# kvignesh1420/rlap

Hardware: AMD Instinct MI355X
Metric: eliminated-vertices/sec (higher is better)
Workload: dtype f64

## Files before the change

### rlap_amd/csrc/rlap_core.h

```cpp
#pragma once
#include <stdint.h>

#if defined(__HIPCC__)
#define RLAP_HD __host__ __device__ __forceinline__
#define RLAP_HD_NOINLINE __host__ __device__ __noinline__
#else
#define RLAP_HD inline
#define RLAP_HD_NOINLINE inline
#endif

namespace rlap {

enum { OV_RANDOM = 0, OV_DEGREE = 1, OV_COARSEN = 2 };
enum { ON_ASC = 0, ON_DESC = 1, ON_RANDOM = 2 };

enum {
    ST_OK = 0,
    ST_NOT_SYMMETRIC = 1,
    ST_INDEX_RANGE = 2,
    ST_BAD_ARG = 3,
    ST_POOL_OVERFLOW = 4,
    ST_LOG_OVERFLOW = 5,
    ST_RNG_OVERFLOW = 6,
    ST_OUT_OVERFLOW = 7,
    ST_HIP_ERROR = 8,
    ST_TOO_LARGE = 9,
    ST_INTERNAL = 10,
    ST_FLOW_SCRATCH = 12,
    ST_FLOW_REORDER = 13,
};

RLAP_HD uint64_t mix64(uint64_t z) {
    z += 0x9E3779B97F4A7C15ull;
    z = (z ^ (z >> 30)) * 0xBF58476D1CE4E5B9ull;
    z = (z ^ (z >> 27)) * 0x94D049BB133111EBull;
    return z ^ (z >> 31);
}
RLAP_HD uint64_t keyed_order_base(uint64_t seed, int64_t vertex, int phase) {
    return mix64(seed ^ mix64(2ull * (uint64_t)vertex + (uint64_t)phase));
}
RLAP_HD uint64_t keyed_order_key(uint64_t base, int64_t nbr) { return mix64(base ^ mix64((uint64_t)nbr)); }

enum { RNG_STREAM = 0, RNG_COUNTER = 1 };
RLAP_HD double frontier_uniform(uint64_t seed, int64_t vertex, int64_t j) {
    const uint64_t z = mix64(mix64((seed ^ 0x66726F6E74696572ull) ^ mix64((uint64_t)vertex)) ^ mix64((uint64_t)j));
    return (double)(z >> 11) * 1.1102230246251565e-16;
}

constexpr int CHUNK0 = 8;
RLAP_HD int ilog2_u32(unsigned q) {
#if defined(__HIP_DEVICE_COMPILE__)
    return 31 - __clz((int)q);
#else
    int c = 0;
    while (q > 1u) { q >>= 1; ++c; }
    return c;
#endif
}
RLAP_HD int chunk_of(int a) {
    return ilog2_u32((unsigned)a / CHUNK0 + 1u);
}
RLAP_HD int chunk_start(int c) { return CHUNK0 * ((1 << c) - 1); }
RLAP_HD int chunk_cap(int c) { return CHUNK0 << c; }

RLAP_HD int pq_list_of(int key, int n) { return key <= n ? key : n + key / n; }

RLAP_HD void pq_op(int& key, int& mv, int n, int delta, int opnum) {
    if (delta < 0 && key == 1) return;
    int ol = pq_list_of(key, n), nl = pq_list_of(key + delta, n);
    key += delta;
    if (ol != nl) mv = opnum;
}

struct SRec {
    double key;
    int32_t idx;
    int32_t aux;
};

template <bool GREATER>
RLAP_HD bool srec_less(const SRec& a, const SRec& b) {
    return GREATER ? (a.key > b.key) : (a.key < b.key);
}

template <class T, class Less, class P>
RLAP_HD void gs_adjust_heap(P a, int first, int hole, int len, T value, Less less) {
    const int top = hole;
    int child = hole;
    while (child < (len - 1) / 2) {
        child = 2 * (child + 1);
        if (less(a[first + child], a[first + child - 1])) child--;
        a[first + hole] = a[first + child];
        hole = child;
    }
    if ((len & 1) == 0 && child == (len - 2) / 2) {
        child = 2 * (child + 1);
        a[first + hole] = a[first + child - 1];
        hole = child - 1;
    }
    int parent = (hole - 1) / 2;
    while (hole > top && less(a[first + parent], value)) {
        a[first + hole] = a[first + parent];
        hole = parent;
        parent = (hole - 1) / 2;
    }
    a[first + hole] = value;
}

template <class T, class Less, class P>
RLAP_HD void gs_heap_sort(P a, int first, int last, Less less) {
    int len = last - first;
    if (len >= 2) {
        int parent = (len - 2) / 2;
        while (true) {
            T v = a[first + parent];
            gs_adjust_heap<T>(a, first, parent, len, v, less);
            if (parent == 0) break;
            parent--;
        }
    }
    int l = last;
    while (l - first > 1) {
        --l;
        T v = a[l];
        a[l] = a[first];
        gs_adjust_heap<T>(a, first, 0, l - first, v, less);
    }
}

template <class T, class Less, class P>
RLAP_HD void gs_introsort_loop(P a, int n, Less less) {
    if (n <= 16) return;
    int depth0 = 0;
    for (unsigned q = (unsigned)n; q > 1u; q >>= 1) ++depth0;
    depth0 *= 2;
    int stk_first[72], stk_last[72], stk_depth[72];
    int sp = 0;
    stk_first[0] = 0; stk_last[0] = n; stk_depth[0] = depth0; sp = 1;
    while (sp > 0) {
        --sp;
        int first = stk_first[sp], last = stk_last[sp], depth = stk_depth[sp];
        while (last - first > 16) {
            if (depth == 0) { gs_heap_sort<T>(a, first, last, less); break; }
            --depth;
            int ia = first + 1, ib = first + (last - first) / 2, ic = last - 1;
            int pick;
            if (less(a[ia], a[ib])) {
                if (less(a[ib], a[ic])) pick = ib;
                else if (less(a[ia], a[ic])) pick = ic;
                else pick = ia;
            } else if (less(a[ia], a[ic])) pick = ia;
            else if (less(a[ib], a[ic])) pick = ic;
            else pick = ib;
            { T t = a[first]; a[first] = a[pick]; a[pick] = t; }
            T pv = a[first];
            int f = first + 1, l = last;
            while (true) {
                while (less(a[f], pv)) ++f;
                --l;
                while (less(pv, a[l])) --l;
                if (!(f < l)) break;
                T t = a[f]; a[f] = a[l]; a[l] = t;
                ++f;
            }
            int cut = f;
            stk_first[sp] = cut; stk_last[sp] = last; stk_depth[sp] = depth; ++sp;
            last = cut;
        }
    }
}

template <class T, class Less, class P>
RLAP_HD void gs_introsort_loop_small(P a, int n, Less less) {
    if (n <= 16) return;
    int depth = 0;
    for (unsigned q = (unsigned)n; q > 1u; q >>= 1) ++depth;
    depth *= 2;
    int first = 0, last = n;
    while (last - first > 16) {
        if (depth == 0) { gs_heap_sort<T>(a, first, last, less); break; }
        --depth;
        int ia = first + 1, ib = first + (last - first) / 2, ic = last - 1;
        int pick;
        if (less(a[ia], a[ib])) {
            if (less(a[ib], a[ic])) pick = ib;
            else if (less(a[ia], a[ic])) pick = ic;
            else pick = ia;
        } else if (less(a[ia], a[ic])) pick = ia;
        else if (less(a[ib], a[ic])) pick = ic;
        else pick = ib;
        { T t = a[first]; a[first] = a[pick]; a[pick] = t; }
        T pv = a[first];
        int f = first + 1, l = last;
        while (true) {
            while (less(a[f], pv)) ++f;
            --l;
            while (less(pv, a[l])) --l;
            if (!(f < l)) break;
            T t = a[f]; a[f] = a[l]; a[l] = t;
            ++f;
        }
        if (last - f > 16) first = f; else last = f;
    }
}
template <class T, class Less, class P>
RLAP_HD void gs_insertion_sort(P a, int n, Less less) {
    for (int i = 1; i < n; ++i) {
        T v = a[i];
        int j = i - 1;
        while (j >= 0 && less(v, a[j])) { a[j + 1] = a[j]; --j; }
        a[j + 1] = v;
    }
}

template <class T, class Less, class P>
RLAP_HD void gs_std_sort_small(P a, int n, Less less) {
    if (n < 2) return;
    gs_introsort_loop_small<T>(a, n, less);
    gs_insertion_sort<T>(a, n, less);
}

template <class T, class Less, class P>
RLAP_HD void gs_std_sort(P a, int n, Less less) {
    if (n < 2) return;
    gs_introsort_loop<T>(a, n, less);
    gs_insertion_sort<T>(a, n, less);
}

template <bool GREATER>
struct SRecLess {
    RLAP_HD bool operator()(const SRec& x, const SRec& y) const { return GREATER ? (x.key > y.key) : (x.key < y.key); }
};

template <bool GREATER, class P>
RLAP_HD void ss_heap_sort(P a, int first, int last) { gs_heap_sort<SRec>(a, first, last, SRecLess<GREATER>()); }

template <bool GREATER, class P>
RLAP_HD void std_sort_emul(P a, int n) { gs_std_sort<SRec>(a, n, SRecLess<GREATER>()); }

RLAP_HD double keyed_order_dkey(uint64_t base, int64_t nbr) { return (double)(keyed_order_key(base, nbr) >> 12); }

struct GraphDesc {
    int32_t vbase;
    int32_t n;
    int64_t t;
    int32_t bucket_base;
    int32_t pad0;
    int32_t pad1;
    int32_t scr_base;
    int32_t scr_cap;
    int32_t minlist;
    int32_t push_cnt;
    int32_t n_elim;
    int32_t status;
    int64_t n_draws;
    int64_t out_rows;
    int32_t flow_base;
    int32_t resume;
    int32_t narrow;
    int32_t narrow_rounds;
    int32_t pool_cur;
    int32_t pool_end;
};

struct ColBuf {
    SRec* rec;
    int32_t* a_slot; int32_t* a_nbr; int32_t* a_twin; double* a_val;
    int32_t* b_slot; int32_t* b_nbr; int32_t* b_twin; double* b_val;
    double* cum; double* newv;
    int32_t* ksel; int32_t* t_key; int32_t* t_mv; int32_t* t_of;
};

struct alignas(16) Slot {
    double val;
    int32_t nbr;
    int32_t twin;
};
struct alignas(16) VRec {
    int32_t key;
    int32_t pqpos;
    int32_t app_cnt;
    int32_t app_chunk;
};
struct Arrays {
    const int32_t* colptr;
    Slot* e;
    int32_t slot_cap;
    int32_t* pool_top;
    VRec* vr;
    int32_t* ocur; int32_t* oend;
    int32_t* bs_cnt; int32_t* bs_alloc;
    int32_t* bs_dir;
    int32_t* bs_v; int32_t* bs_id;
    int32_t* bs_pool_top; int32_t bs_pool_cap;
    const int32_t* orig_order;
    const double* rng; int64_t rng_len;
    const int64_t* perm;
    int32_t o_v; int32_t o_n;
    uint64_t shuffle_seed;
    int32_t rng_mode;
    int32_t vbase;
};
RLAP_HD double arr_uniform(const Arrays& A, int64_t draw, int32_t vertex, int32_t j) {
    return A.rng_mode == RNG_COUNTER ? frontier_uniform(A.shuffle_seed, (int64_t)(vertex - A.vbase), (int64_t)j) : A.rng[draw];
}
RLAP_HD bool keyed_order(const Arrays& A) { return A.o_n == ON_RANDOM || A.o_v == OV_COARSEN; }

#if defined(__HIP_DEVICE_COMPILE__)
RLAP_HD int32_t pool_take(int32_t* top, int32_t cnt) { return atomicAdd(top, cnt); }
#else
RLAP_HD int32_t pool_take(int32_t* top, int32_t cnt) { int32_t r = *top; *top = r + cnt; return r; }
#endif

RLAP_HD int32_t col_append(const Arrays& A, int32_t k) {
    int32_t a = A.vr[k].app_cnt;
    int c = chunk_of(a);
    int cs = chunk_start(c);
    if (a == cs) {
        int32_t need = 1 + chunk_cap(c);
        int32_t base = pool_take(A.pool_top, need);
        if (base < 0 || base > A.slot_cap - need) return -1;
        A.e[base].nbr = A.vr[k].app_chunk;
        A.vr[k].app_chunk = base;
    }
    A.vr[k].app_cnt = a + 1;
    return A.vr[k].app_chunk + 1 + (a - cs);
}

RLAP_HD int32_t serial_gather(const Arrays& A, int32_t v, const ColBuf& B, int32_t cap) {
    int32_t len = 0;
    int32_t a = A.vr[v].app_cnt;
    if (a > 0) {
        int32_t base = A.vr[v].app_chunk;
        int c = chunk_of(a - 1);
        int32_t idx = a - 1;
        while (idx >= 0) {
            int32_t cs = chunk_start(c);
            for (int32_t t = idx; t >= cs; --t) {
                int32_t s = base + 1 + (t - cs);
                double val = A.e[s].val;
                if (val > 0) {
                    if (len < cap) { B.a_slot[len] = s; B.a_nbr[len] = A.e[s].nbr; B.a_val[len] = val; B.a_twin[len] = A.e[s].twin; }
                    ++len;
                }
            }
            idx = cs - 1;
            base = A.e[base].nbr;
            --c;
        }
    }
    for (int32_t s = A.colptr[v + 1] - 1; s >= A.colptr[v]; --s) {
        double val = A.e[s].val;
        if (val > 0) {
            if (len < cap) { B.a_slot[len] = s; B.a_nbr[len] = A.e[s].nbr; B.a_val[len] = val; B.a_twin[len] = A.e[s].twin; }
            ++len;
        }
    }
    return len;
}

constexpr int SQUEEZE_PASSES = 2;

template <class F>
RLAP_HD void col_for_each_slot(const Arrays& A, int32_t v, F f) {
    const int32_t a = A.vr[v].app_cnt;
    if (a > 0) {
        int32_t base = A.vr[v].app_chunk;
        int c = chunk_of(a - 1);
        int32_t idx = a - 1;
        while (idx >= 0 && base >= 0) {
            const int32_t cs = chunk_start(c);
            for (int32_t t = idx; t >= cs; --t) f(base + 1 + (t - cs));
            idx = cs - 1;
            base = A.e[base].nbr;
            --c;
        }
    }
    for (int32_t s = A.colptr[v + 1] - 1; s >= A.colptr[v]; --s) f(s);
}
#if defined(__HIPCC__)
template <class Sink>
__device__ __forceinline__ int32_t wave_col_live(const Arrays& A, int32_t v, int lane, Sink sink) {
    const uint64_t lt = lane == 0 ? 0ull : (~0ull >> (64 - lane));
    int32_t len = 0;
    auto piece = [&](int32_t hi, int32_t lo) {
        for (int32_t s0 = hi; s0 >= lo; s0 -= 64) {
            const int32_t s = s0 - lane;
            Slot g = {};
            if (s >= lo) g = A.e[s];
            const bool live = s >= lo && g.val > 0;
            const uint64_t mask = __ballot(live);
            if (live) sink(len + __popcll(mask & lt), s, g);
            len += __popcll(mask);
        }
    };
    const int32_t cp0 = A.colptr[v], cp1 = A.colptr[v + 1];
    int32_t idx = A.vr[v].app_cnt - 1, base = A.vr[v].app_chunk;
    for (int c = idx >= 0 ? chunk_of(idx) : 0; idx >= 0; --c) {
        const int32_t cs = chunk_start(c);
        piece(base + 1 + (idx - cs), base + 1);
        idx = cs - 1; base = A.e[base].nbr;
    }
    piece(cp1 - 1, cp0);
    return len;
}
#endif
RLAP_HD int32_t squeeze_rank_col(const Arrays& A, int32_t v, int32_t* rank) {
    int32_t r = 0;
    col_for_each_slot(A, v, [&](int32_t s) { if (A.e[s].val > 0) rank[s] = r++; });
    return r;
}
RLAP_HD int32_t squeeze_slot(const int32_t* colptr2, int32_t col, int32_t r) { return colptr2[col + 1] - 1 - r; }
RLAP_HD bool squeeze_entry(const Arrays& A, const int32_t* rank, const int32_t* colptr2, Slot* e2, int32_t n_total, int32_t v, int32_t s) {
    const Slot x = A.e[s];
    if ((uint32_t)x.nbr >= (uint32_t)n_total || (uint32_t)x.twin >= (uint32_t)A.slot_cap) return false;
    const int32_t d = squeeze_slot(colptr2, v, rank[s]);
    if (d < colptr2[v] || d >= colptr2[v + 1]) return false;
    Slot y;
    y.val = x.val; y.nbr = x.nbr; y.twin = squeeze_slot(colptr2, x.nbr, rank[x.twin]);
    e2[d] = y;
    return true;
}

constexpr int BCH0 = 16;
constexpr int BDIR = 26;
RLAP_HD int bs_chunk_of(int a) { return ilog2_u32((unsigned)a / BCH0 + 1u); }
RLAP_HD int bs_chunk_start(int c) { return BCH0 * ((1 << c) - 1); }
RLAP_HD int bs_chunk_cap(int c) { return BCH0 << c; }
RLAP_HD int32_t bs_slot(const Arrays& A, int32_t b, int32_t a) {
    int c = bs_chunk_of(a);
    return A.bs_dir[(int64_t)b * BDIR + c] + (a - bs_chunk_start(c));
}
RLAP_HD bool bs_ensure(const Arrays& A, int32_t b, int32_t a) {
    int c = bs_chunk_of(a);
    int32_t have = A.bs_alloc[b];
    while (have <= c) {
        int32_t need = bs_chunk_cap(have);
        int32_t base = pool_take(A.bs_pool_top, need);
        if (base < 0 || base > A.bs_pool_cap - need) return false;
        A.bs_dir[(int64_t)b * BDIR + have] = base;
        ++have;
    }
    A.bs_alloc[b] = have;
    return true;
}

RLAP_HD int pq_push(const Arrays& A, GraphDesc& G, int32_t v, int32_t lst) {
    int32_t b = G.bucket_base + lst;
    int32_t a = A.bs_cnt[b];
    if (!bs_ensure(A, b, a)) return ST_LOG_OVERFLOW;
    int32_t s = bs_slot(A, b, a);
    int32_t id = G.push_cnt++;
    A.bs_v[s] = v; A.bs_id[s] = id;
    A.bs_cnt[b] = a + 1;
    A.vr[v].pqpos = id;
    if (lst < G.minlist) G.minlist = lst;
    return ST_OK;
}

RLAP_HD int32_t pq_pop(const Arrays& A, GraphDesc& G) {
    while (true) {
        int32_t b = G.bucket_base + G.minlist;
        int32_t cnt = A.bs_cnt[b];
        while (cnt > 0) {
            int32_t s = bs_slot(A, b, cnt - 1);
            --cnt;
            int32_t v = A.bs_v[s];
            if (A.vr[v].pqpos == A.bs_id[s]) { A.bs_cnt[b] = cnt; A.vr[v].pqpos = -2; return v; }
        }
        A.bs_cnt[b] = 0;
        int32_t oc = A.ocur[b], oe = A.oend[b];
        while (oc < oe) {
            int32_t v = A.orig_order[oc++];
            if (A.vr[v].pqpos == -1) { A.ocur[b] = oc; A.vr[v].pqpos = -2; return v; }
        }
        A.ocur[b] = oc;
        G.minlist += 1;
        if (G.minlist > 2 * G.n) return -1;
    }
}

RLAP_HD int pq_commit_serial(const Arrays& A, GraphDesc& G, const ColBuf& B, int32_t m) {
    int32_t cnt = 0;
    for (int32_t x = 0; x < m; ++x) {
        A.vr[B.b_nbr[x]].key = B.t_key[x];
        if (B.t_mv[x] >= 0) { B.rec[cnt].key = (double)B.t_mv[x]; B.rec[cnt].idx = x; B.rec[cnt].aux = 0; ++cnt; }
    }
    std_sort_emul<false>(B.rec, cnt);
    for (int32_t i = 0; i < cnt; ++i) {
        int32_t x = B.rec[i].idx;
        int rc = pq_push(A, G, B.b_nbr[x], pq_list_of(B.t_key[x], G.n));
        if (rc) return rc;
    }
    return ST_OK;
}

RLAP_HD int32_t serial_sort_merge(const Arrays& A, const GraphDesc& G, const ColBuf& B, int32_t len0, bool elim, bool use_pq) {
    for (int32_t i = 0; i < len0; ++i) { B.rec[i].key = (double)B.a_nbr[i]; B.rec[i].idx = i; B.rec[i].aux = 0; }
    std_sort_emul<false>(B.rec, len0);
    int32_t m = 0;
    for (int32_t i = 0; i < len0; ++i) {
        int32_t s = B.rec[i].idx;
        if (m == 0 || B.a_nbr[s] != B.b_nbr[m - 1]) {
            B.b_slot[m] = B.a_slot[s]; B.b_nbr[m] = B.a_nbr[s]; B.b_val[m] = B.a_val[s]; B.b_twin[m] = B.a_twin[s];
            if (elim && use_pq) { B.t_key[m] = A.vr[B.a_nbr[s]].key; B.t_mv[m] = -1; }
            ++m;
        } else {
            B.b_val[m - 1] += B.a_val[s];
            if (elim) {
                A.e[B.a_twin[s]].val = 0;
                if (use_pq) pq_op(B.t_key[m - 1], B.t_mv[m - 1], G.n, -1, i);
            }
        }
    }
    return m;
}

RLAP_HD void serial_order(const Arrays& A, const ColBuf& B, int32_t m, int32_t vertex, int phase, int32_t vbase) {
    if (A.o_n == ON_RANDOM || A.o_v == OV_COARSEN) {
        uint64_t base = keyed_order_base(A.shuffle_seed, vertex - vbase, phase);
        for (int32_t i = 0; i < m; ++i) { B.rec[i].key = keyed_order_dkey(base, B.b_nbr[i] - vbase); B.rec[i].idx = i; B.rec[i].aux = 0; }
        std_sort_emul<false>(B.rec, m);
    } else {
        for (int32_t i = 0; i < m; ++i) { B.rec[i].key = B.b_val[i]; B.rec[i].idx = i; B.rec[i].aux = 0; }
        if (A.o_n == ON_ASC) std_sort_emul<false>(B.rec, m); else std_sort_emul<true>(B.rec, m);
    }
    for (int32_t j = 0; j < m; ++j) {
        int32_t x = B.rec[j].idx;
        B.t_of[j] = x;
        B.a_slot[j] = B.b_slot[x]; B.a_nbr[j] = B.b_nbr[x]; B.a_val[j] = B.b_val[x]; B.a_twin[j] = B.b_twin[x];
    }
}

RLAP_HD int32_t upper_index(const double* cum, int32_t m, double r) {
    int32_t lo = 0, hi = m;
    while (lo < hi) {
        int32_t mid = (lo + hi) >> 1;
        if (cum[mid] > r) hi = mid; else lo = mid + 1;
    }
    return lo < m ? lo : m - 1;
}

RLAP_HD int serial_rewire(const Arrays& A, int32_t s_r, int32_t nbr_j, int32_t k, double w) {
    int32_t s_n = col_append(A, k);
    if (s_n < 0) return ST_POOL_OVERFLOW;
    A.e[s_r].nbr = k; A.e[s_r].val = w; A.e[s_r].twin = s_n;
    A.e[s_n].nbr = nbr_j; A.e[s_n].val = w; A.e[s_n].twin = s_r;
    return ST_OK;
}

RLAP_HD int serial_eliminate(const Arrays& A, GraphDesc& G, const ColBuf& B, int32_t cap, int32_t v, int64_t e1) {
    const bool use_pq = A.o_v != OV_RANDOM;
    int32_t len0 = serial_gather(A, v, B, cap);
    if (len0 > cap) return ST_INTERNAL;
    int32_t m = serial_sort_merge(A, G, B, len0, true, use_pq);
    serial_order(A, B, m, v, 0, G.vbase);
    if (A.o_v == OV_COARSEN) {
        if (m >= 1) {
            double csum = 0;
            for (int32_t j = 0; j < m; ++j) { csum += B.a_val[j]; B.cum[j] = csum; }
            if (A.rng_mode != RNG_COUNTER && G.n_draws >= A.rng_len) return ST_RNG_OVERFLOW;
            double u = arr_uniform(A, G.n_draws, v, 0); G.n_draws += 1;
            double r = u * csum;
            int32_t koff = upper_index(B.cum, m, r);
            int32_t k = B.a_nbr[koff];
            double wk = B.a_val[koff];
            A.e[B.a_twin[koff]].val = 0;
            int32_t xk = B.t_of[koff];
            pq_op(B.t_key[xk], B.t_mv[xk], G.n, -1, len0);
            for (int32_t j = 0; j < m; ++j) {
                if (j == koff) continue;
                pq_op(B.t_key[xk], B.t_mv[xk], G.n, +1, len0 + 1 + j);
                double w = B.a_val[j];
                double nw = (wk * w) / (wk + w);
                int rc = serial_rewire(A, B.a_twin[j], B.a_nbr[j], k, nw);
                if (rc) return rc;
            }
        }
    } else {
        double csum = 0;
        for (int32_t j = 0; j < m; ++j) { csum += B.a_val[j]; B.cum[j] = csum; }
        if (A.rng_mode != RNG_COUNTER && m > 1 && G.n_draws + (m - 1) > A.rng_len) return ST_RNG_OVERFLOW;
        double wdeg = csum, colScale = 1;
        for (int32_t j = 0; j < m - 1; ++j) {
            double w = B.a_val[j] * colScale;
            double f = w / wdeg;
            double u = arr_uniform(A, G.n_draws + j, v, j);
            double r = u * (csum - B.cum[j]) + B.cum[j];
            int32_t koff = upper_index(B.cum, m, r);
            B.ksel[j] = koff;
            double omf = 1 - f;
            B.newv[j] = f * omf * wdeg;
            colScale = colScale * omf;
            wdeg = wdeg * omf * omf;
        }
        if (m > 1) G.n_draws += m - 1;
        for (int32_t j = 0; j < m - 1; ++j) {
            int32_t koff = B.ksel[j];
            if (use_pq) { int32_t xk = B.t_of[koff]; pq_op(B.t_key[xk], B.t_mv[xk], G.n, +1, len0 + j); }
            int rc = serial_rewire(A, B.a_twin[j], B.a_nbr[j], B.a_nbr[koff], B.newv[j]);
            if (rc) return rc;
        }
        if (m > 0) {
            if (use_pq && e1 + 1 < (int64_t)G.n) { int32_t xl = B.t_of[m - 1]; pq_op(B.t_key[xl], B.t_mv[xl], G.n, -1, len0 + m); }
            A.e[B.a_twin[m - 1]].val = 0;
        }
    }
    if (use_pq) return pq_commit_serial(A, G, B, m);
    return ST_OK;
}

RLAP_HD int32_t serial_output(const Arrays& A, const GraphDesc& G, const ColBuf& B, int32_t cap, int32_t v, double* out, int64_t row0, bool count_only) {
    int32_t len0 = serial_gather(A, v, B, cap);
    if (len0 > cap) return -1;
    int32_t m = serial_sort_merge(A, G, B, len0, false, false);
    if (count_only) return m;
    serial_order(A, B, m, v, 1, G.vbase);
    for (int32_t j = 0; j < m; ++j) {
        double* o = out + 3 * (row0 + j);
        o[0] = (double)B.a_nbr[j]; o[1] = (double)v; o[2] = B.a_val[j];
    }
    return m;
}


constexpr int BCAP = 32;

struct TRes {
    int32_t key_after;
    int16_t mv;
    uint8_t c;
    uint8_t flags;
};
struct Ent {
    double val;
    union {
        double aux;
        TRes res;
    };
    int32_t nbr;
    int32_t twin;
};
enum { CF_BIG = 1, CF_DUP = 2, CF_COMPLEX = 4, CF_DEP = 8, CF_TIE = 16, CF_NEQ = 32, CF_READY = 64, CF_PATCHED = 128 };
constexpr int DEPMAX = 4;
enum { TF_CONTENDED = 1 };

template <int BC> struct CandPad {};
template <> struct CandPad<64> { int64_t pad64; };
template <> struct CandPad<128> { int64_t pad128; };
template <int BC>
struct CandT : CandPad<BC> {
    static constexpr int CAP = BC;
    Ent e[BC];
    uint8_t ksel[BC];
    int32_t v;
    int32_t m;
    int32_t flags;
    int32_t src;
    int32_t ndraw;
    int32_t koff;
    int32_t cp1;
    int32_t acnt;
    int32_t ext;
    int32_t nmv;
    int32_t nkill;
    int32_t cb[BC <= 16 ? 2 : (BC <= 32 ? 3 : (BC <= 64 ? 4 : 5))];
    int32_t ndep;
    uint8_t dep[4];
    int64_t draw0;
};
static_assert(sizeof(CandT<16>) == 472 && sizeof(CandT<32>) == 872, "record sizes the LDS budget of the round kernel is counted with");
typedef CandT<BCAP> Cand;

RLAP_HD TRes& ent_tres(Ent& e) { return e.res; }

struct EntLessNbr { RLAP_HD bool operator()(const Ent& x, const Ent& y) const { return x.nbr < y.nbr; } };
struct EntLessVal { RLAP_HD bool operator()(const Ent& x, const Ent& y) const { return x.val < y.val; } };
struct EntGreaterVal { RLAP_HD bool operator()(const Ent& x, const Ent& y) const { return x.val > y.val; } };
struct EntLessAux { RLAP_HD bool operator()(const Ent& x, const Ent& y) const { return x.aux < y.aux; } };

struct KI { double k; uint8_t idx; };
struct KIRef {
    Ent* e; uint8_t* ix; int i;
    RLAP_HD operator KI() const { KI v; v.k = e[i].aux; v.idx = ix[i]; return v; }
    RLAP_HD KIRef& operator=(const KI& v) { e[i].aux = v.k; ix[i] = v.idx; return *this; }
    RLAP_HD KIRef& operator=(const KIRef& o) { KI v = o; e[i].aux = v.k; ix[i] = v.idx; return *this; }
};
struct KIArr {
    Ent* e; uint8_t* ix;
    RLAP_HD KIRef operator[](int i) const { KIRef r; r.e = e; r.ix = ix; r.i = i; return r; }
};
struct KILess { RLAP_HD bool operator()(const KI& x, const KI& y) const { return x.k < y.k; } };
struct KIGreater { RLAP_HD bool operator()(const KI& x, const KI& y) const { return x.k > y.k; } };

template <class CT>
RLAP_HD void cand_order_index(const Arrays& A, CT& C) {
    const int32_t m = C.m;
    for (int32_t j = 0; j < m; ++j) C.ksel[j] = (uint8_t)j;
    KIArr arr; arr.e = C.e; arr.ix = C.ksel;
    if (CT::CAP <= 32) {
        if (A.o_n == ON_DESC && A.o_v != OV_COARSEN) gs_std_sort_small<KI>(arr, m, KIGreater());
        else gs_std_sort_small<KI>(arr, m, KILess());
    } else {
        if (A.o_n == ON_DESC && A.o_v != OV_COARSEN) gs_std_sort<KI>(arr, m, KIGreater());
        else gs_std_sort<KI>(arr, m, KILess());
    }
    C.ndraw = (A.o_v == OV_COARSEN) ? (m >= 1 ? 1 : 0) : (m > 1 ? m - 1 : 0);
}

template <class CT>
RLAP_HD bool cand_merges_multi_edges(const Arrays& A) { return CT::CAP >= 64 && A.o_v == OV_RANDOM; }

template <class CT>
RLAP_HD void cand_meta(const Arrays& A, int32_t v, CT& C) {
    C.v = v; C.flags = 0; C.m = 0; C.ndraw = 0; C.koff = 0; C.nkill = 0; C.nmv = 0; C.ndep = 0;
    int32_t cp0 = A.colptr[v], cp1 = A.colptr[v + 1];
    int32_t acnt = A.vr[v].app_cnt;
    int32_t base = A.vr[v].app_chunk;
    C.cp1 = cp1; C.acnt = acnt; C.ext = (cp1 - cp0) + acnt;
    if (C.ext > CT::CAP) { C.flags = CF_BIG; C.ext = 0; return; }
    if (acnt > 0) {
        int ct = chunk_of(acnt - 1);
        for (int c = ct; c >= 0; --c) { C.cb[c] = base; if (c > 0) base = A.e[base].nbr; }
    }
}
template <class CT>
RLAP_HD int32_t cand_slot(const CT& C, int32_t e) {
    if (e < C.acnt) {
        int32_t a = C.acnt - 1 - e;
        int c = chunk_of(a);
        return C.cb[c] + 1 + (a - chunk_start(c));
    }
    return C.cp1 - 1 - (e - C.acnt);
}
template <class CT>
RLAP_HD void cand_load(const Arrays& A, CT& C, int32_t e) {
    int32_t s = cand_slot(C, e);
    C.e[e].val = A.e[s].val; C.e[e].nbr = A.e[s].nbr; C.e[e].twin = A.e[s].twin; C.e[e].aux = 0;
}
template <class CT>
RLAP_HD void cand_finish(const Arrays& A, CT& C, int32_t vbase = 0) {
    if (C.flags & CF_BIG) return;
    int32_t len = 0;
    for (int32_t e = 0; e < C.ext; ++e) {
        if (C.e[e].val > 0) { if (len != e) C.e[len] = C.e[e]; ++len; }
    }
    C.m = len;
    gs_std_sort<Ent>(C.e, len, EntLessNbr());
    if (cand_merges_multi_edges<CT>(A)) {
        int32_t mm = 0, nk = 0;
        int32_t kill[CT::CAP];
        for (int32_t i = 0; i < len; ++i) {
            if (mm == 0 || C.e[i].nbr != C.e[mm - 1].nbr) { if (mm != i) C.e[mm] = C.e[i]; ++mm; }
            else { C.e[mm - 1].val += C.e[i].val; kill[nk++] = C.e[i].twin; }
        }
        for (int32_t q = 0; q < nk; ++q) C.e[mm + q].twin = kill[q];
        C.nkill = nk;
        len = mm;
        C.m = len;
    } else {
        for (int32_t i = 1; i < len; ++i) if (C.e[i].nbr == C.e[i - 1].nbr) { C.flags = CF_DUP; return; }
    }
    if (A.o_n == ON_RANDOM || A.o_v == OV_COARSEN) {
        uint64_t kb = keyed_order_base(A.shuffle_seed, C.v - vbase, 0);
        for (int32_t i = 0; i < len; ++i) C.e[i].aux = keyed_order_dkey(kb, C.e[i].nbr - vbase);
        gs_std_sort<Ent>(C.e, len, EntLessAux());
    } else if (A.o_n == ON_ASC) {
        gs_std_sort<Ent>(C.e, len, EntLessVal());
    } else {
        gs_std_sort<Ent>(C.e, len, EntGreaterVal());
    }
    C.ndraw = (A.o_v == OV_COARSEN) ? (len >= 1 ? 1 : 0) : (len > 1 ? len - 1 : 0);
}
template <class CT>
RLAP_HD void cand_prepare(const Arrays& A, int32_t v, CT& C, int32_t vbase = 0) {
    cand_meta(A, v, C);
    for (int32_t e = 0; e < C.ext; ++e) cand_load(A, C, e);
    cand_finish(A, C, vbase);
}

template <class CT>
RLAP_HD bool cand_patch(const Arrays& A, CT* cand, int32_t d, int32_t vbase) {
    CT& C = cand[d];
    if (C.nkill > 0) return false;
    for (int32_t q = 0; q < C.ndep; ++q) {
        const int32_t j = C.dep[q];
        const CT& J = cand[j];
        int32_t p = -1;
        for (int32_t z = 0; z < J.m; ++z) if (J.e[z].nbr == C.v) p = z;
        if (p < 0 || p == J.m - 1) return false;
        for (int32_t z = 0; z < J.m - 1; ++z) if (J.ksel[z] == p) return false;
        if (!(J.e[p].val > 0)) return false;
        const int32_t k = J.e[J.ksel[p]].nbr;
        int32_t qd = -1;
        for (int32_t z = 0; z < C.m; ++z) { if (C.e[z].nbr == J.v) qd = z; if (C.e[z].nbr == k) { C.flags |= CF_DUP; return false; } }
        if (qd < 0) return false;
        C.e[qd].nbr = k; C.e[qd].val = J.e[p].val; C.e[qd].twin = ~(j * CT::CAP + p);
    }
    C.flags |= CF_PATCHED;
    const int32_t len = C.m;
    gs_std_sort<Ent>(C.e, len, EntLessNbr());
    if (A.o_n == ON_RANDOM || A.o_v == OV_COARSEN) {
        uint64_t kb = keyed_order_base(A.shuffle_seed, C.v - vbase, 0);
        for (int32_t i = 0; i < len; ++i) C.e[i].aux = keyed_order_dkey(kb, C.e[i].nbr - vbase);
        gs_std_sort<Ent>(C.e, len, EntLessAux());
    } else if (A.o_n == ON_ASC) {
        gs_std_sort<Ent>(C.e, len, EntLessVal());
    } else {
        gs_std_sort<Ent>(C.e, len, EntGreaterVal());
    }
    return true;
}

RLAP_HD int32_t ent_upper_index(const Ent* e, int32_t m, double r) {
    int32_t lo = 0, hi = m;
    while (lo < hi) {
        int32_t mid = (lo + hi) >> 1;
        if (e[mid].aux > r) hi = mid; else lo = mid + 1;
    }
    return lo < m ? lo : m - 1;
}

template <class CT>
RLAP_HD void cand_cumsum(const Arrays& A, CT& C) {
    const int32_t m = C.m;
    double csum = 0;
    for (int32_t j = 0; j < m; ++j) { csum += C.e[j].val; C.e[j].aux = csum; }
    if (A.o_v == OV_COARSEN && m >= 1) {
        double u = arr_uniform(A, C.draw0, C.v, 0);
        double r = u * csum;
        int32_t koff = ent_upper_index(C.e, m, r);
        C.koff = koff;
        double wk = C.e[koff].val;
        for (int32_t j = 0; j < m; ++j) {
            if (j == koff) continue;
            double w = C.e[j].val;
            C.e[j].val = (wk * w) / (wk + w);
            C.ksel[j] = (uint8_t)koff;
        }
    }
}
template <class CT>
RLAP_HD void cand_pick(const Arrays& A, CT& C, int32_t j) {
    const int32_t m = C.m;
    double csum = C.e[m - 1].aux;
    double u = arr_uniform(A, C.draw0 + j, C.v, j);
    double cj = C.e[j].aux;
    double r = u * (csum - cj) + cj;
    C.ksel[j] = (uint8_t)ent_upper_index(C.e, m, r);
}
template <class CT>
RLAP_HD void cand_recur(const Arrays& A, CT& C) {
    if (A.o_v == OV_COARSEN) return;
    const int32_t m = C.m;
    if (m < 1) return;
    double wdeg = C.e[m - 1].aux, colScale = 1;
    for (int32_t j = 0; j < m - 1; ++j) {
        double w = C.e[j].val * colScale;
        double f = w / wdeg;
        double omf = 1 - f;
        C.e[j].val = f * omf * wdeg;
        colScale = colScale * omf;
        wdeg = wdeg * omf * omf;
    }
}
template <class CT>
RLAP_HD void cand_sample(const Arrays& A, CT& C) {
    cand_cumsum(A, C);
    if (A.o_v != OV_COARSEN) for (int32_t j = 0; j < C.m - 1; ++j) cand_pick(A, C, j);
    cand_recur(A, C);
}

RLAP_HD int popcount_u64(uint64_t x) {
#if defined(__HIP_DEVICE_COMPILE__)
    return __popcll(x);
#else
    return __builtin_popcountll(x);
#endif
}
RLAP_HD int clz_u64(uint64_t x) {
#if defined(__HIP_DEVICE_COMPILE__)
    return __clzll((long long)x);
#else
    return __builtin_clzll(x);
#endif
}
RLAP_HD int ctz_u64(uint64_t x) {
#if defined(__HIP_DEVICE_COMPILE__)
    return __ffsll((long long)x) - 1;
#else
    return __builtin_ctzll(x);
#endif
}
RLAP_HD uint64_t ksel_matches(const uint8_t* ksel, int32_t w, int32_t j, int32_t limit) {
    const uint64_t lo7 = 0x7F7F7F7F7F7F7F7Full;
    const uint64_t x = reinterpret_cast<const uint64_t*>(ksel)[w] ^ (0x0101010101010101ull * (uint64_t)(uint8_t)j);
    uint64_t y = ~(((x & lo7) + lo7) | x | lo7);
    const int32_t valid = limit - 8 * w;
    if (valid < 8) y &= valid <= 0 ? 0ull : ((1ull << (8 * valid)) - 1ull);
    return y;
}
template <class CT>
RLAP_HD void cand_replay_pre(const Arrays& A, const CT& C, int32_t j, int* cnt, int* last_inc) {
    const int32_t m = C.m;
    int32_t li = -1, c = 0;
    if (A.o_v == OV_COARSEN) {
        if (j == C.koff) c = m - 1;
    } else {
        for (int32_t w = 0; 8 * w < m - 1; ++w) {
            const uint64_t y = ksel_matches(C.ksel, w, j, m - 1);
            if (y) { c += popcount_u64(y); li = 8 * w + ((63 - clz_u64(y)) >> 3); }
        }
    }
    *cnt = c; *last_inc = li;
}
RLAP_HD bool cand_touches(int o_v, int32_t m, int32_t j, int32_t koff, int c) {
    if (o_v == OV_COARSEN) return j == koff;
    return c > 0 || j == m - 1;
}
template <class CT>
RLAP_HD int32_t cand_replay_post(const Arrays& A, const CT& C, int32_t j, int32_t key0, int32_t n, bool allow_last_dec,
                                 int c, int last_inc, int* mv, bool* complex) {
    const int32_t m = C.m;
    int32_t key = key0;
    *mv = -1;
    if (A.o_v == OV_COARSEN) {
        if (j == C.koff) {
            if (key != 1) { key -= 1; *mv = m; }
            if (c > 0) {
                key += c;
                int32_t lastj = (C.koff == m - 1) ? m - 2 : m - 1;
                *mv = m + 1 + lastj;
            }
        }
    } else {
        if (c > 0) { key += c; *mv = m + last_inc; }
        if (j == m - 1 && allow_last_dec && key != 1) { key -= 1; *mv = 2 * m; }
    }
    if (key0 > n || key0 + c > n) *complex = true;
    return key;
}
template <class CT>
RLAP_HD int32_t cand_replay(const Arrays& A, const CT& C, int32_t j, int32_t key0, int32_t n, bool allow_last_dec,
                            int* mv, int* cnt, bool* complex) {
    int c, li;
    cand_replay_pre(A, C, j, &c, &li);
    *cnt = c;
    return cand_replay_post(A, C, j, key0, n, allow_last_dec, c, li, mv, complex);
}

}
```

### rlap_amd/csrc/rlap_squeeze.h

```cpp
#pragma once
#include <hip/hip_runtime.h>
#include <stdint.h>

#include "rlap_core.h"

namespace rlap {

constexpr int SQ_SHORT = 64;

struct SqueezeBufs {
    int passes;
    Slot* e2;
    int32_t* colptr2;
    int32_t* rank;
    int32_t* cnt;
    int32_t* longlist;
    int32_t* nlong;
    int32_t* marks;
    const int32_t* vgraph;
    void* scan_tmp; size_t scan_tmp_bytes;
    int32_t N;
};

int squeeze_scan_tmp_bytes(int64_t N, size_t* bytes);

int launch_squeeze(hipStream_t stream, const Arrays& A, const SqueezeBufs& Q, int pass, Slot* e_dst, int32_t* colptr_dst, GraphDesc* gd, int32_t G,
                   const int32_t* in_flags, const double* in_acc);

}
```

### rlap_amd/csrc/rlap_squeeze.hip

```cpp
#include <algorithm>
#include <cstring>

#include <hip/hip_runtime.h>
#include <rocprim/rocprim.hpp>

#include "rlap_core.h"
#include "rlap_kernels.h"
#include "rlap_squeeze.h"

namespace rlap {

namespace {

__device__ __forceinline__ bool sq_bad_input(const int32_t* __restrict__ in_flags, const double* __restrict__ in_acc) {
    return in_flags[FLAG_RANGE] || in_flags[FLAG_CROSS] || in_flags[FLAG_PERM] || in_acc[2] != 0.0 || !(in_acc[0] <= 1e-24 * in_acc[1]);
}

template <class F>
__device__ __forceinline__ void wave_col_slots(const Arrays& A, int32_t v, int lane, F f) {
    auto piece = [&](int32_t hi, int32_t lo) {
        for (int32_t s0 = hi; s0 >= lo; s0 -= 64) { const int32_t s = s0 - lane; f(s, s >= lo); }
    };
    const int32_t a = A.vr[v].app_cnt;
    if (a > 0) {
        int32_t base = A.vr[v].app_chunk;
        int c = chunk_of(a - 1);
        int32_t idx = a - 1;
        while (idx >= 0 && base >= 0 && base < A.slot_cap) {
            const int32_t cs = chunk_start(c);
            piece(base + 1 + (idx - cs), base + 1);
            idx = cs - 1;
            base = A.e[base].nbr;
            --c;
        }
    }
    piece(A.colptr[v + 1] - 1, A.colptr[v]);
}

__global__ __launch_bounds__(256) void k_sq_rank(Arrays A, int32_t N, const int32_t* __restrict__ vgraph, const GraphDesc* __restrict__ gd,
                                                 const int32_t* __restrict__ in_flags, const double* __restrict__ in_acc,
                                                 int32_t* __restrict__ rank, int32_t* __restrict__ cnt, int32_t* __restrict__ longlist,
                                                 int32_t* __restrict__ nlong) {
    const int32_t v = blockIdx.x * blockDim.x + threadIdx.x;
    if (v > N) return;
    if (v == N) { cnt[N] = 0; return; }
    int32_t c = 0;
    if (A.vr[v].pqpos != -2 && !sq_bad_input(in_flags, in_acc) && gd[vgraph[v]].status == 0) {
        const int32_t ext = (A.colptr[v + 1] - A.colptr[v]) + A.vr[v].app_cnt;
        if (ext > SQ_SHORT) { longlist[atomicAdd(nlong, 1)] = v; return; }
        c = squeeze_rank_col(A, v, rank);
    }
    cnt[v] = c;
}

__global__ __launch_bounds__(256) void k_sq_rank_long(Arrays A, const int32_t* __restrict__ longlist, const int32_t* __restrict__ nlong,
                                                      int32_t* __restrict__ rank, int32_t* __restrict__ cnt) {
    const int lane = threadIdx.x & 63;
    const int32_t nw = (int32_t)(gridDim.x * (blockDim.x >> 6));
    const int32_t n = *nlong;
    for (int32_t i = (int32_t)(blockIdx.x * (blockDim.x >> 6) + (threadIdx.x >> 6)); i < n; i += nw) {
        const int32_t v = longlist[i];
        int32_t run = 0;
        wave_col_slots(A, v, lane, [&](int32_t s, bool valid) {
            const bool live = valid && A.e[s].val > 0;
            const unsigned long long m = __ballot(live);
            if (live) rank[s] = run + __popcll(m & ((1ull << lane) - 1ull));
            run += __popcll(m);
        });
        if (lane == 0) cnt[v] = run;
    }
}

__global__ __launch_bounds__(256) void k_sq_copy(Arrays A, int32_t N, const int32_t* __restrict__ vgraph, GraphDesc* __restrict__ gd,
                                                 const int32_t* __restrict__ rank, const int32_t* __restrict__ colptr2, Slot* __restrict__ e2) {
    const int32_t v = blockIdx.x * blockDim.x + threadIdx.x;
    if (v >= N) return;
    if (colptr2[v + 1] == colptr2[v]) return;
    if ((A.colptr[v + 1] - A.colptr[v]) + A.vr[v].app_cnt > SQ_SHORT) return;
    bool ok = true;
    col_for_each_slot(A, v, [&](int32_t s) { if (A.e[s].val > 0) ok &= squeeze_entry(A, rank, colptr2, e2, N, v, s); });
    if (!ok) atomicMax(&gd[vgraph[v]].status, (int32_t)ST_INTERNAL);
}

__global__ __launch_bounds__(256) void k_sq_copy_long(Arrays A, int32_t N, const int32_t* __restrict__ vgraph, GraphDesc* __restrict__ gd,
                                                      const int32_t* __restrict__ longlist, const int32_t* __restrict__ nlong,
                                                      const int32_t* __restrict__ rank, const int32_t* __restrict__ colptr2, Slot* __restrict__ e2) {
    const int lane = threadIdx.x & 63;
    const int32_t nw = (int32_t)(gridDim.x * (blockDim.x >> 6));
    const int32_t n = *nlong;
    for (int32_t i = (int32_t)(blockIdx.x * (blockDim.x >> 6) + (threadIdx.x >> 6)); i < n; i += nw) {
        const int32_t v = longlist[i];
        bool ok = true;
        wave_col_slots(A, v, lane, [&](int32_t s, bool valid) { if (valid && A.e[s].val > 0) ok &= squeeze_entry(A, rank, colptr2, e2, N, v, s); });
        if (!ok) atomicMax(&gd[vgraph[v]].status, (int32_t)ST_INTERNAL);
    }
}

__global__ __launch_bounds__(256) void k_sq_epilogue(VRec* __restrict__ vr, int32_t N, const int32_t* __restrict__ colptr2, int32_t* __restrict__ pool_top,
                                                     GraphDesc* __restrict__ gd, int32_t G, int32_t* __restrict__ marks) {
    const int32_t i = blockIdx.x * blockDim.x + threadIdx.x;
    if (i < N) { vr[i].app_cnt = 0; vr[i].app_chunk = -1; }
    if (i < G) { gd[i].pool_cur = 0; gd[i].pool_end = 0; gd[i].narrow = 0; marks[i] = gd[i].narrow_rounds; }
    if (i == 0) *pool_top = colptr2[N];
}

}

int squeeze_scan_tmp_bytes(int64_t N, size_t* bytes) {
    size_t b = 0;
    hipError_t e = rocprim::exclusive_scan(nullptr, b, (int32_t*)nullptr, (int32_t*)nullptr, (int32_t)0, (size_t)(N + 1), rocprim::plus<int32_t>(), (hipStream_t) nullptr);
    *bytes = b;
    return (int)e;
}

int launch_squeeze(hipStream_t stream, const Arrays& A, const SqueezeBufs& Q, int pass, Slot* e_dst, int32_t* colptr_dst, GraphDesc* gd, int32_t G,
                   const int32_t* in_flags, const double* in_acc) {
    const int32_t N = Q.N;
    const unsigned nb = (unsigned)((N + 1 + 255) / 256);
    const unsigned nb_long = 1024;
    hipError_t e = hipMemsetAsync(Q.nlong, 0, sizeof(int32_t), stream);
    if (e != hipSuccess) return (int)e;
    hipLaunchKernelGGL(k_sq_rank, dim3(nb), dim3(256), 0, stream, A, N, Q.vgraph, gd, in_flags, in_acc, Q.rank, Q.cnt, Q.longlist, Q.nlong);
    hipLaunchKernelGGL(k_sq_rank_long, dim3(nb_long), dim3(256), 0, stream, A, Q.longlist, Q.nlong, Q.rank, Q.cnt);
    size_t bytes = Q.scan_tmp_bytes;
    e = rocprim::exclusive_scan(Q.scan_tmp, bytes, Q.cnt, colptr_dst, (int32_t)0, (size_t)(N + 1), rocprim::plus<int32_t>(), stream);
    if (e != hipSuccess) return (int)e;
    hipLaunchKernelGGL(k_sq_copy, dim3(nb), dim3(256), 0, stream, A, N, Q.vgraph, gd, Q.rank, colptr_dst, e_dst);
    hipLaunchKernelGGL(k_sq_copy_long, dim3(nb_long), dim3(256), 0, stream, A, N, Q.vgraph, gd, Q.longlist, Q.nlong, Q.rank, colptr_dst, e_dst);
    const unsigned nbe = (unsigned)((std::max<int32_t>(N, G) + 255) / 256);
    hipLaunchKernelGGL(k_sq_epilogue, dim3(nbe), dim3(256), 0, stream, A.vr, N, colptr_dst, A.pool_top, gd, G, Q.marks + (size_t)pass * (size_t)G);
    return (int)hipGetLastError();
}

}
```

Measured before the change: 2.139 million.

## Process short squeeze columns with sub-wave lane groups instead of one thread

The short-column rank and copy kernels now assign a group of GS lanes (8 by default, 4 or 16 via RLAP_SQ_GROUP) to each vertex instead of one thread. The group leader resolves the column's chunk bases once and broadcasts them with shuffles, then the lanes walk positions in strides and compute ranks with ballot masks and popcount. This is meant to cut per-thread serial walks and uncoalesced loads on skewed short columns. In exchange it launches GS times more threads, and groups whose columns are shorter than GS leave lanes idle.

```diff
diff --git a/rlap_amd/csrc/rlap_core.h b/rlap_amd/csrc/rlap_core.h
--- a/rlap_amd/csrc/rlap_core.h
+++ b/rlap_amd/csrc/rlap_core.h
@@ -411,16 +411,70 @@
     return r;
 }
 RLAP_HD int32_t squeeze_slot(const int32_t* colptr2, int32_t col, int32_t r) { return colptr2[col + 1] - 1 - r; }
-RLAP_HD bool squeeze_entry(const Arrays& A, const int32_t* rank, const int32_t* colptr2, Slot* e2, int32_t n_total, int32_t v, int32_t s) {
-    const Slot x = A.e[s];
+RLAP_HD bool squeeze_entry_ranked(const Arrays& A, const int32_t* rank, const int32_t* colptr2, Slot* e2, int32_t n_total, int32_t v, const Slot& x, int32_t r) {
     if ((uint32_t)x.nbr >= (uint32_t)n_total || (uint32_t)x.twin >= (uint32_t)A.slot_cap) return false;
-    const int32_t d = squeeze_slot(colptr2, v, rank[s]);
+    const int32_t d = squeeze_slot(colptr2, v, r);
     if (d < colptr2[v] || d >= colptr2[v + 1]) return false;
     Slot y;
     y.val = x.val; y.nbr = x.nbr; y.twin = squeeze_slot(colptr2, x.nbr, rank[x.twin]);
     e2[d] = y;
     return true;
 }
+RLAP_HD bool squeeze_entry(const Arrays& A, const int32_t* rank, const int32_t* colptr2, Slot* e2, int32_t n_total, int32_t v, int32_t s) {
+    return squeeze_entry_ranked(A, rank, colptr2, e2, n_total, v, A.e[s], rank[s]);
+}
+
+constexpr int SQ_SHORT = 64;
+constexpr int SQ_CHUNKS = 4;
+static_assert(CHUNK0 * ((1 << SQ_CHUNKS) - 1) >= SQ_SHORT && CHUNK0 * ((1 << (SQ_CHUNKS - 1)) - 1) < SQ_SHORT, "SQ_CHUNKS chunks hold SQ_SHORT appended entries");
+struct SqCol {
+    int32_t a;
+    int32_t cp0, cp1;
+    int32_t cb0, cb1, cb2, cb3;
+};
+RLAP_HD int32_t sq_col_ext(const SqCol& C) { return C.a + (C.cp1 - C.cp0); }
+RLAP_HD SqCol sq_col_resolve(const Slot* e, int32_t slot_cap, int32_t cp0, int32_t cp1, int32_t a, int32_t chunk) {
+    SqCol C;
+    C.a = a > 0 ? a : 0; C.cp0 = cp0; C.cp1 = cp1; C.cb0 = -1; C.cb1 = -1; C.cb2 = -1; C.cb3 = -1;
+    if (C.a + (cp1 - cp0) > SQ_SHORT || cp1 < cp0) { C.a = 0; C.cp1 = cp0; return C; }
+    if (C.a > 0) {
+        const int ctop = chunk_of(C.a - 1);
+        int32_t base = chunk;
+        bool ok = true;
+#if defined(__HIP_DEVICE_COMPILE__)
+#pragma unroll
+#endif
+        for (int c = SQ_CHUNKS - 1; c >= 0; --c) {
+            if (c > ctop) continue;
+            ok = ok && base >= 0 && base < slot_cap;
+            if (!ok) break;
+            if (c == 3) C.cb3 = base; else if (c == 2) C.cb2 = base; else if (c == 1) C.cb1 = base; else C.cb0 = base;
+            if (c > 0) base = e[base].nbr;
+        }
+    }
+    return C;
+}
+RLAP_HD int32_t sq_pos_slot(const SqCol& C, int32_t slot_cap, int32_t p) {
+    if (p < 0 || p >= sq_col_ext(C)) return -1;
+    if (p >= C.a) return C.cp1 - 1 - (p - C.a);
+    const int32_t t = C.a - 1 - p;
+    const int c = chunk_of(t);
+    const int32_t base = c == 0 ? C.cb0 : (c == 1 ? C.cb1 : (c == 2 ? C.cb2 : C.cb3));
+    if (base < 0) return -1;
+    const int32_t s = base + 1 + (t - chunk_start(c));
+    return s < slot_cap ? s : -1;
+}
+RLAP_HD int32_t sq_group_pos(int g, int l, int32_t turn) { return turn * g + l; }
+RLAP_HD int32_t sq_group_turns(int g, int32_t ext) { return (ext + g - 1) / g; }
+RLAP_HD uint32_t sq_group_mask(uint64_t wave_mask, int lane, int g) { return (uint32_t)(wave_mask >> (lane & ~(g - 1))) & ((1u << g) - 1u); }
+RLAP_HD int sq_popc(uint32_t x) {
+#if defined(__HIP_DEVICE_COMPILE__)
+    return __popc(x);
+#else
+    return __builtin_popcount(x);
+#endif
+}
+RLAP_HD int32_t sq_group_rank(uint32_t gm, int l, int32_t run) { return run + sq_popc(gm & ((1u << l) - 1u)); }
 
 constexpr int BCH0 = 16;
 constexpr int BDIR = 26;
diff --git a/rlap_amd/csrc/rlap_squeeze.h b/rlap_amd/csrc/rlap_squeeze.h
--- a/rlap_amd/csrc/rlap_squeeze.h
+++ b/rlap_amd/csrc/rlap_squeeze.h
@@ -6,7 +6,7 @@
 
 namespace rlap {
 
-constexpr int SQ_SHORT = 64;
+constexpr int SQ_GROUP = 8;
 
 struct SqueezeBufs {
     int passes;
diff --git a/rlap_amd/csrc/rlap_squeeze.hip b/rlap_amd/csrc/rlap_squeeze.hip
--- a/rlap_amd/csrc/rlap_squeeze.hip
+++ b/rlap_amd/csrc/rlap_squeeze.hip
@@ -1,4 +1,5 @@
 #include <algorithm>
+#include <cstdlib>
 #include <cstring>
 
 #include <hip/hip_runtime.h>
@@ -37,20 +38,46 @@
     piece(A.colptr[v + 1] - 1, A.colptr[v]);
 }
 
+constexpr SqCol SQ_NO_COL = {0, 0, 0, -1, -1, -1, -1};
+template <int GS>
+__device__ __forceinline__ SqCol group_bcast(SqCol C, int lane) {
+    const int lead = lane & ~(GS - 1);
+    C.a = __shfl(C.a, lead); C.cp0 = __shfl(C.cp0, lead); C.cp1 = __shfl(C.cp1, lead);
+    C.cb0 = __shfl(C.cb0, lead); C.cb1 = __shfl(C.cb1, lead); C.cb2 = __shfl(C.cb2, lead); C.cb3 = __shfl(C.cb3, lead);
+    return C;
+}
+
+template <int GS>
 __global__ __launch_bounds__(256) void k_sq_rank(Arrays A, int32_t N, const int32_t* __restrict__ vgraph, const GraphDesc* __restrict__ gd,
                                                  const int32_t* __restrict__ in_flags, const double* __restrict__ in_acc,
                                                  int32_t* __restrict__ rank, int32_t* __restrict__ cnt, int32_t* __restrict__ longlist,
                                                  int32_t* __restrict__ nlong) {
-    const int32_t v = blockIdx.x * blockDim.x + threadIdx.x;
-    if (v > N) return;
-    if (v == N) { cnt[N] = 0; return; }
-    int32_t c = 0;
-    if (A.vr[v].pqpos != -2 && !sq_bad_input(in_flags, in_acc) && gd[vgraph[v]].status == 0) {
-        const int32_t ext = (A.colptr[v + 1] - A.colptr[v]) + A.vr[v].app_cnt;
-        if (ext > SQ_SHORT) { longlist[atomicAdd(nlong, 1)] = v; return; }
-        c = squeeze_rank_col(A, v, rank);
-    }
-    cnt[v] = c;
+    const int lane = threadIdx.x & 63, l = lane & (GS - 1);
+    const int64_t v64 = ((int64_t)blockIdx.x * blockDim.x + threadIdx.x) / GS;
+    const int32_t v = (int32_t)(v64 < (int64_t)N ? v64 : (int64_t)N);
+    const bool lead = l == 0 && v64 < (int64_t)N;
+    SqCol C = SQ_NO_COL;
+    bool is_long = false;
+    if (l == 0 && v64 == (int64_t)N) cnt[N] = 0;
+    if (lead) {
+        const VRec r = A.vr[v];
+        if (r.pqpos != -2 && !sq_bad_input(in_flags, in_acc) && gd[vgraph[v]].status == 0) {
+            const int32_t cp0 = A.colptr[v], cp1 = A.colptr[v + 1];
+            if ((cp1 - cp0) + r.app_cnt > SQ_SHORT) { longlist[atomicAdd(nlong, 1)] = v; is_long = true; }
+            else C = sq_col_resolve(A.e, A.slot_cap, cp0, cp1, r.app_cnt, r.app_chunk);
+        }
+    }
+    C = group_bcast<GS>(C, lane);
+    const int32_t ext = sq_col_ext(C);
+    int32_t run = 0;
+    for (int32_t k = 0; __ballot(k * GS < ext) != 0ull; ++k) {
+        const int32_t s = sq_pos_slot(C, A.slot_cap, sq_group_pos(GS, l, k));
+        const bool live = s >= 0 && A.e[s].val > 0;
+        const uint32_t gm = sq_group_mask(__ballot(live), lane, GS);
+        if (live) rank[s] = sq_group_rank(gm, l, run);
+        run += sq_popc(gm);
+    }
+    if (lead && !is_long) cnt[v] = run;
 }
 
 __global__ __launch_bounds__(256) void k_sq_rank_long(Arrays A, const int32_t* __restrict__ longlist, const int32_t* __restrict__ nlong,
@@ -71,14 +98,31 @@
     }
 }
 
+template <int GS>
 __global__ __launch_bounds__(256) void k_sq_copy(Arrays A, int32_t N, const int32_t* __restrict__ vgraph, GraphDesc* __restrict__ gd,
                                                  const int32_t* __restrict__ rank, const int32_t* __restrict__ colptr2, Slot* __restrict__ e2) {
-    const int32_t v = blockIdx.x * blockDim.x + threadIdx.x;
-    if (v >= N) return;
-    if (colptr2[v + 1] == colptr2[v]) return;
-    if ((A.colptr[v + 1] - A.colptr[v]) + A.vr[v].app_cnt > SQ_SHORT) return;
+    const int lane = threadIdx.x & 63, l = lane & (GS - 1);
+    const int64_t v64 = ((int64_t)blockIdx.x * blockDim.x + threadIdx.x) / GS;
+    const int32_t v = (int32_t)(v64 < (int64_t)N ? v64 : (int64_t)N);
+    SqCol C = SQ_NO_COL;
+    if (l == 0 && v64 < (int64_t)N && colptr2[v + 1] != colptr2[v]) {
+        const VRec r = A.vr[v];
+        const int32_t cp0 = A.colptr[v], cp1 = A.colptr[v + 1];
+        if ((cp1 - cp0) + r.app_cnt <= SQ_SHORT) C = sq_col_resolve(A.e, A.slot_cap, cp0, cp1, r.app_cnt, r.app_chunk);
+    }
+    C = group_bcast<GS>(C, lane);
+    const int32_t ext = sq_col_ext(C);
+    int32_t run = 0;
     bool ok = true;
-    col_for_each_slot(A, v, [&](int32_t s) { if (A.e[s].val > 0) ok &= squeeze_entry(A, rank, colptr2, e2, N, v, s); });
+    for (int32_t k = 0; __ballot(k * GS < ext) != 0ull; ++k) {
+        const int32_t s = sq_pos_slot(C, A.slot_cap, sq_group_pos(GS, l, k));
+        Slot x = {};
+        if (s >= 0) x = A.e[s];
+        const bool live = s >= 0 && x.val > 0;
+        const uint32_t gm = sq_group_mask(__ballot(live), lane, GS);
+        if (live) ok &= squeeze_entry_ranked(A, rank, colptr2, e2, N, v, x, sq_group_rank(gm, l, run));
+        run += sq_popc(gm);
+    }
     if (!ok) atomicMax(&gd[vgraph[v]].status, (int32_t)ST_INTERNAL);
 }
 
@@ -113,19 +157,40 @@
     return (int)e;
 }
 
+namespace {
+int squeeze_group() {
+    if (const char* e = std::getenv("RLAP_SQ_GROUP")) { const int q = std::atoi(e); if (q == 4 || q == 8 || q == 16) return q; }
+    return SQ_GROUP;
+}
+template <int GS>
+void launch_short_rank(hipStream_t stream, const Arrays& A, const SqueezeBufs& Q, const GraphDesc* gd, const int32_t* in_flags, const double* in_acc) {
+    const unsigned nb = (unsigned)((((int64_t)Q.N + 1) * GS + 255) / 256);
+    hipLaunchKernelGGL(k_sq_rank<GS>, dim3(nb), dim3(256), 0, stream, A, Q.N, Q.vgraph, gd, in_flags, in_acc, Q.rank, Q.cnt, Q.longlist, Q.nlong);
+}
+template <int GS>
+void launch_short_copy(hipStream_t stream, const Arrays& A, const SqueezeBufs& Q, GraphDesc* gd, const int32_t* colptr_dst, Slot* e_dst) {
+    const unsigned nb = (unsigned)((((int64_t)Q.N + 1) * GS + 255) / 256);
+    hipLaunchKernelGGL(k_sq_copy<GS>, dim3(nb), dim3(256), 0, stream, A, Q.N, Q.vgraph, gd, Q.rank, colptr_dst, e_dst);
+}
+}
+
 int launch_squeeze(hipStream_t stream, const Arrays& A, const SqueezeBufs& Q, int pass, Slot* e_dst, int32_t* colptr_dst, GraphDesc* gd, int32_t G,
                    const int32_t* in_flags, const double* in_acc) {
     const int32_t N = Q.N;
-    const unsigned nb = (unsigned)((N + 1 + 255) / 256);
+    const int gs = squeeze_group();
     const unsigned nb_long = 1024;
     hipError_t e = hipMemsetAsync(Q.nlong, 0, sizeof(int32_t), stream);
     if (e != hipSuccess) return (int)e;
-    hipLaunchKernelGGL(k_sq_rank, dim3(nb), dim3(256), 0, stream, A, N, Q.vgraph, gd, in_flags, in_acc, Q.rank, Q.cnt, Q.longlist, Q.nlong);
+    if (gs == 4) launch_short_rank<4>(stream, A, Q, gd, in_flags, in_acc);
+    else if (gs == 16) launch_short_rank<16>(stream, A, Q, gd, in_flags, in_acc);
+    else launch_short_rank<8>(stream, A, Q, gd, in_flags, in_acc);
     hipLaunchKernelGGL(k_sq_rank_long, dim3(nb_long), dim3(256), 0, stream, A, Q.longlist, Q.nlong, Q.rank, Q.cnt);
     size_t bytes = Q.scan_tmp_bytes;
     e = rocprim::exclusive_scan(Q.scan_tmp, bytes, Q.cnt, colptr_dst, (int32_t)0, (size_t)(N + 1), rocprim::plus<int32_t>(), stream);
     if (e != hipSuccess) return (int)e;
-    hipLaunchKernelGGL(k_sq_copy, dim3(nb), dim3(256), 0, stream, A, N, Q.vgraph, gd, Q.rank, colptr_dst, e_dst);
+    if (gs == 4) launch_short_copy<4>(stream, A, Q, gd, colptr_dst, e_dst);
+    else if (gs == 16) launch_short_copy<16>(stream, A, Q, gd, colptr_dst, e_dst);
+    else launch_short_copy<8>(stream, A, Q, gd, colptr_dst, e_dst);
     hipLaunchKernelGGL(k_sq_copy_long, dim3(nb_long), dim3(256), 0, stream, A, N, Q.vgraph, gd, Q.longlist, Q.nlong, Q.rank, colptr_dst, e_dst);
     const unsigned nbe = (unsigned)((std::max<int32_t>(N, G) + 255) / 256);
     hipLaunchKernelGGL(k_sq_epilogue, dim3(nbe), dim3(256), 0, stream, A.vr, N, colptr_dst, A.pool_top, gd, G, Q.marks + (size_t)pass * (size_t)G);
```

Result: no change. 2.157 million (median of 6 runs) (+0.9%).
